# norabelrose/sparse-vae

Measured on AMD Instinct MI355X. Metric: training tokens/sec + ELBO match vs CPU ref, 512-tok seq, 1/2/4/8 MI355X, higher is better.
Workload: dtype bf16; 1 GPU; c2: TransformerVAE 6L d512 heads 8 seq 512, batch 64/GPU, dense attention, dropout 0.1, fwd+bwd+allreduce+clip+RAdam; model=TransformerVAE-6L-d512, global_batch=64, seq_len=512, parallelism=dp1

## Files before the change

sparse-vae_amd/csrc/gemm.hip:

```cpp
#include "common.h"
#include "../../include/svae.h"
#include <string.h>
#include <algorithm>
#include <vector>

using namespace svae;

namespace {

constexpr int BM = 128, BN = 128, BK = 64;
constexpr int TILE_BYTES = BM * BK * 2;

struct GP {
  const bf16* A; const bf16* B;
  long long lda, ldb, sA, sB;
  int M, N, K, splits, kchunk, tiles_n, tiles_m;
  void* C; long long ldc, sC;
  const float* bias;
  const float* resid; long long ldr;
  void* aux; long long ldaux;
  float alpha, drop_p;
  unsigned long long seed;
  const float* rot_tab; int rot_cols, rot_d, rot_seq;
  const int* labels; float* label_logit;
// ... 615 lines not shown

template <bool NT = false>
__device__ __forceinline__ void store_pair_bf16(bf16* row_base, int colbase, int ncols_left, const f32x4& x,
                                                const f32x4& y, int g) {
  const unsigned x0 = pack_bf16x2(x[0], x[1]), x1 = pack_bf16x2(x[2], x[3]);
  const unsigned y0 = pack_bf16x2(y[0], y[1]), y1 = pack_bf16x2(y[2], y[3]);
  const auto s0 = __builtin_amdgcn_permlane16_swap(x0, y0, false, false);
  const auto s1 = __builtin_amdgcn_permlane16_swap(x1, y1, false, false);
  const int c = colbase + ((g & 1) ? 16 : 0) + ((g & 2) ? 8 : 0);
  const u32x4 w = {s0[0], s1[0], s0[1], s1[1]};
  if (c + 8 <= ncols_left) {
    if constexpr (NT) __builtin_nontemporal_store(w, (u32x4*)(row_base + c));
    else *(u32x4*)(row_base + c) = w;
  } else if (c < ncols_left) *(u32x2*)(row_base + c) = (u32x2){w[0], w[1]};
}

template <bool B>
struct BoolC {
  static constexpr bool value = B;
};

template <int EPI>
__device__ __forceinline__ void g3_reg_epilogue(const GP& p, const f32x4 (&acc)[8][4], const float* sbias,
                                                const int* slabel, float* sstat, int m0, int n0, int bn, int batch,
                                                int split, int wr, int wc, int tid, int lane) {
  const long long cofs = (long long)batch * p.sC + split * p.slab;
  const int g = lane >> 4, li = lane & 15;
  f32x4 b4[4];
#pragma unroll
  for (int j = 0; j < 4; ++j) b4[j] = *(const f32x4*)(sbias + wc * 64 + j * 16 + 4 * g);
  f32x4 bl4[4];
#pragma unroll
  for (int j = 0; j < 4; ++j) bl4[j] = b4[j] * G3_LOG2E;
  int rofs[4] = {0, 0, 0, 0};
  bool rot_on[4] = {false, false, false, false};
  int pos = 0, pstep = 0;
  f32x4 cs_cur[4], cs_nxt[4];
  auto rot_load = [&](int ps, f32x4 (&cs)[4]) {
    const float* t = p.rot_tab + (long long)ps * p.rot_d;
#pragma unroll
    for (int j = 0; j < 4; ++j) cs[j] = rot_on[j] ? *(const f32x4*)(t + rofs[j]) : (f32x4){1.f, 0.f, 1.f, 0.f};
  };
  if constexpr (EPI == SVAE_EPI_ROTARY_BF16) {
#pragma unroll
    for (int j = 0; j < 4; ++j) {
      const int n = n0 + wc * 64 + j * 16 + 4 * g;
      rot_on[j] = n < p.rot_cols;
      rofs[j] = ((n % p.rot_d) >> 1) * 2;
    }
    pos = (m0 + wr * 128 + li) % p.rot_seq;
    pstep = 16 % p.rot_seq;
    rot_load(pos, cs_cur);
  }
#pragma unroll
  for (int i = 0; i < 8; ++i) {
    const int rl = wr * 128 + i * 16 + li, m = m0 + rl;
    f32x4 v[4];
#pragma unroll
    for (int j = 0; j < 4; ++j) v[j] = p.alpha * acc[i][j] + b4[j];
    if constexpr (EPI == SVAE_EPI_ROTARY_BF16) {
      int pn = pos + pstep;
      if (pn >= p.rot_seq) pn -= p.rot_seq;
      if (i + 1 < 8) rot_load(pn, cs_nxt);
#pragma unroll
      for (int j = 0; j < 4; ++j) {
        const f32x4 cs2 = cs_cur[j];
        const float a0 = v[j][0], b0 = v[j][1], a1 = v[j][2], b1 = v[j][3];
        v[j][0] = a0 * cs2[0] + (-b0) * cs2[1];
        v[j][1] = b0 * cs2[0] + a0 * cs2[1];
        v[j][2] = a1 * cs2[2] + (-b1) * cs2[3];
        v[j][3] = b1 * cs2[2] + a1 * cs2[3];
      }
      pos = pn;
      if (i + 1 < 8) {
#pragma unroll
        for (int j = 0; j < 4; ++j) cs_cur[j] = cs_nxt[j];
      }
    }
    {
      if constexpr (EPI == SVAE_EPI_GELU) {
        f32x4 gg[4], dg[4];
#pragma unroll
        for (int j = 0; j < 4; ++j)
#pragma unroll
          for (int e = 0; e < 4; e += 2) {
            f32x2 ge, de;
            gelu_pair2((f32x2){v[j][e], v[j][e + 1]}, ge, de);
            gg[j][e] = ge[0];
            gg[j][e + 1] = ge[1];
            dg[j][e] = de[0];
            dg[j][e + 1] = de[1];
          }
        store_rows_bf16<false>((bf16*)p.C + cofs, p.ldc, m0 + wr * 128 + i * 16, p.M, n0 + wc * 64, p.N, gg, g, li);
        store_rows_bf16<true>((bf16*)p.aux, p.ldaux, m0 + wr * 128 + i * 16, p.M, n0 + wc * 64, p.N, dg, g, li);
      } else if constexpr (EPI == SVAE_EPI_CE_PROB) {
        const float off = sstat[1024 + rl] * G3_LOG2E;
        const f32x2 sa2 = {p.alpha * G3_LOG2E, p.alpha * G3_LOG2E}, noff = {-off, -off};
        f32x2 se2 = {0.f, 0.f};
        auto body = [&](auto rag) {
          f32x4 xs[4];
#pragma unroll
          for (int j = 0; j < 4; ++j)
#pragma unroll
              for (int e = 0; e < 4; e += 2) {
                const f32x2 a2 = {acc[i][j][e], acc[i][j][e + 1]};
                const f32x2 c2 = (f32x2){bl4[j][e], bl4[j][e + 1]} + noff;
                const f32x2 t2 = a2 * sa2 + c2;
                f32x2 x = {__builtin_amdgcn_exp2f(t2[0]), __builtin_amdgcn_exp2f(t2[1])};
                if constexpr (decltype(rag)::value) {
                  const int n = n0 + wc * 64 + j * 16 + 4 * g + e;
                  if (n >= p.N) x[0] = 0.f;
                  if (n + 1 >= p.N) x[1] = 0.f;
                }
                xs[j][e] = x[0];
                xs[j][e + 1] = x[1];
                se2 += x;
              }
          store_rows_bf16<true>((bf16*)p.C + cofs, p.ldc, m0 + wr * 128 + i * 16, p.M, n0 + wc * 64, p.N, xs, g, li);
        };
        if (__builtin_amdgcn_readfirstlane((int)(n0 + wc * 64 + 64 > p.N))) body(BoolC<true>{});
        else body(BoolC<false>{});
        float se = sum_x16_x32(se2[0] + se2[1]);
        if (g == 0) sstat[rl * 4 + wc] = se;
      } else if (EPI != SVAE_EPI_CE_STATS || p.C) {
        store_rows_bf16<EPI == SVAE_EPI_CE_STATS>((bf16*)p.C + cofs, p.ldc, m0 + wr * 128 + i * 16, p.M, n0 + wc * 64,
                                                  p.N, v, g, li);
      }
    }
    if constexpr (EPI == SVAE_EPI_CE_STATS) {
      const bool ragged = n0 + wc * 64 + 64 > p.N;
      float mx = -INFINITY;
#pragma unroll
      for (int j = 0; j < 4; ++j)
#pragma unroll
        for (int e = 0; e < 4; ++e) {
          if (ragged && n0 + wc * 64 + j * 16 + 4 * g + e >= p.N) v[j][e] = -INFINITY;
          mx = fmaxf(mx, v[j][e]);
        }
      mx = max_x16_x32(mx);
      const float mc = mx == -INFINITY ? 0.f : mx * G3_LOG2E;
      float se = 0.f;
#pragma unroll
      for (int j = 0; j < 4; ++j)
#pragma unroll
        for (int e = 0; e < 4; ++e) se += __builtin_amdgcn_exp2f(fmaf(v[j][e], G3_LOG2E, -mc));
      se = sum_x16_x32(se);
      if (g == 0) {
        sstat[(rl * 4 + wc) * 2] = mx;
        sstat[(rl * 4 + wc) * 2 + 1] = se;
// ... 188 lines not shown
        const int n = nb + j * 16 + 4 * g;
        r[j] = (ld && m < p.M && n < p.N) ? *(const f32x4*)(src + (long long)m * lds_ + n) : (f32x4){0.f, 0.f, 0.f, 0.f};
      }
    };
    f32x4 cur[4], nxt[4];
    if constexpr (EPI != G3_EPI_SLAB) ld_row(0, cur);
#pragma unroll
    for (int i = 0; i < 8; ++i) {
      if (EPI != G3_EPI_SLAB && i + 1 < 8) ld_row(i + 1, nxt);
      const int m = m0 + wr * 128 + i * 16 + li;
      f32x4 x[4];
#pragma unroll
      for (int j = 0; j < 4; ++j) {
        const int n = nb + j * 16 + 4 * g;
        x[j] = p.alpha * acc[i][j] + b4[j];
        if constexpr (EPI == SVAE_EPI_DROPOUT_RESID) {
          if (p.drop_p > 0.f) dropout4(p, x[j], m, n);
        }
        if constexpr (EPI != G3_EPI_SLAB) x[j] += cur[j];
      }
      if constexpr (EPI == SVAE_EPI_F32_ACC) {
#pragma unroll
        for (int j = 0; j < 4; ++j) {
          const int n = nb + j * 16 + 4 * g;
          if (m < p.M && n < p.N) *(f32x4*)((float*)p.C + cofs + (long long)m * p.ldc + n) = x[j];
        }
      } else {
        store_rows_f32((float*)p.C + cofs, p.ldc, m0 + wr * 128 + i * 16, p.M, nb, p.N, x, g, li);
        if constexpr (EPI == SVAE_EPI_DROPOUT_RESID) {
          if (p.aux) store_rows_bf16<false>((bf16*)p.aux, p.ldaux, m0 + wr * 128 + i * 16, p.M, nb, p.N, x, g, li);
        } else if constexpr (EPI == SVAE_EPI_F32) {
          if (p.aux) {
            if (p.drop_p > 0.f) {
#pragma unroll
              for (int j = 0; j < 4; ++j) dropout4(p, x[j], m, nb + j * 16 + 4 * g);
            }
            store_rows_bf16<false>((bf16*)p.aux, p.ldaux, m0 + wr * 128 + i * 16, p.M, nb, p.N, x, g, li);
          }
        }
      }
      if (EPI != G3_EPI_SLAB && i + 1 < 8) {
#pragma unroll
        for (int j = 0; j < 4; ++j) cur[j] = nxt[j];
      }
    }
  }
}

struct G3Tile {
  int m0, n0, bn, batch, split, kbeg, kend, nk;
  const bf16* A; const bf16* B;
};

__device__ __forceinline__ G3Tile g3_tile(const GP& p, int t3) {
  G3Tile T;
  const int tiles = p.tn2 * p.tm2;
  const int z = t3 / tiles, t = t3 - z * tiles;
  T.batch = z / p.splits;
  T.split = z - T.batch * p.splits;
  int bm, bn;
  group_tile(t, p.tm2, p.tn2, p.group, bm, bn);
  T.bn = bn;
  T.m0 = bm * 256;
  T.n0 = bn * 256;
  T.kbeg = T.split * p.kchunk;
  T.kend = min(p.K, T.kbeg + p.kchunk);
  T.nk = T.kend > T.kbeg ? (T.kend - T.kbeg + 63) / 64 : 0;
  T.A = p.A + T.batch * p.sA;
  T.B = p.B + T.batch * p.sB;
  return T;
}

constexpr int G3_EPI_STORES = 16;

#ifdef SVAE_STAMPS
__device__ unsigned long long svae_stamps[8][96][3];
__device__ unsigned long long svae_rt[1024][2];
#define G3_STAMP(k) \
  do { if (blockIdx.x < 8 && tid == 0 && ntile < 96) svae_stamps[blockIdx.x][ntile][k] = __builtin_amdgcn_s_memtime(); } while (0)
#else
#define G3_STAMP(k) ((void)0)
#endif
#ifndef SVAE_KW_PRE
#define SVAE_KW_PRE 1
#endif

template <int EPI>
constexpr int g3_epi_vmem_ops() {
  switch (EPI) {
    case SVAE_EPI_BF16:
    case G3_EPI_BF16_DELTA:
    case SVAE_EPI_ROTARY_BF16:
    case SVAE_EPI_CE_STATS:
    case SVAE_EPI_ROWSCALE_GATHER:
    case SVAE_EPI_GELU_BWD:
      return 8 * 2;
    case SVAE_EPI_CE_PROB:
      return 8 * 2 + 1;
    case SVAE_EPI_GELU:
      return 8 * 2 * 2;
    case SVAE_EPI_F32:
    case SVAE_EPI_F32_ACC:
    case SVAE_EPI_DROPOUT_RESID:
    case G3_EPI_ACC_KW:
    case G3_EPI_F32_KW:
    case G3_EPI_SLAB:
      return 8 * 4;
    default:
      return 0;
  }
}

template <bool AT, bool BT, int EPI>
__device__ __forceinline__ void gemm256_run(const GP& p, int blk, int nwg, bool remap = true) {
  static_assert(g3_epi_vmem_ops<EPI>() >= G3_EPI_STORES, "the relaxed first wait would not cover the prefetch DMA");
  constexpr bool IS_KW = EPI == G3_EPI_ACC_KW || EPI == G3_EPI_F32_KW;
  __shared__ __attribute__((aligned(16))) char ring[2 * G3_STAGE + 2048 + 8192];
  float* sbias = (float*)(ring + 2 * G3_STAGE);
  int* slabel = (int*)(ring + 2 * G3_STAGE + 1024);
  float* sstat = (float*)(ring + 2 * G3_STAGE + 2048);
  const int tid = threadIdx.x, lane = tid & 63;
  const int wave = __builtin_amdgcn_readfirstlane(tid >> 6);
  const int wr = wave >> 2, wc = wave & 3;
  int bid = blk;
  if (remap && nwg >= 16) {
    const int q = nwg / 8, r = nwg % 8, xcd = bid % 8, idx = bid / 8;
    bid = (xcd < r ? xcd * (q + 1) : r * (q + 1) + (xcd - r) * q) + idx;
  }
  int t3 = bid;
  if (t3 >= p.total3) return;
  G3Tile T = g3_tile(p, t3);
  const G3Src sa = g3_src<AT>(p.lda, wave, lane), sb = g3_src<BT>(p.ldb, wave, lane);
  int g = 0;
  if (T.nk > 0) g3_issue<AT, BT>(p, T.A, T.B, sa, sb, T.m0, T.n0, T.kbeg, T.kend, ring, wave);

  bool relaxed = false;
  int ntile = 0;
  (void)ntile;
  while (true) {
    G3_STAMP(0);
    const int t3n = t3 + nwg;
    const bool has_next = t3n < p.total3;
    float rsum[4] = {0.f, 0.f, 0.f, 0.f};
    f32x4 acc[8][4];
#pragma unroll
    for (int i = 0; i < 8; ++i)
#pragma unroll
      for (int j = 0; j < 4; ++j) acc[i][j] = (f32x4){0.f, 0.f, 0.f, 0.f};

    const bool next_dma = has_next && g3_tile(p, t3n).nk > 0;
    for (int kt = 0; kt < T.nk; ++kt, ++g) {
      if (kt == 0 && relaxed) asm volatile("s_waitcnt vmcnt(%0)" ::"n"(G3_EPI_STORES) : "memory");
      else asm volatile("s_waitcnt vmcnt(0)" ::: "memory");
      __builtin_amdgcn_s_barrier();
      const char* la = ring + (g & 1) * G3_STAGE;
      const char* lb = la + G3_T;
      char* nxt = ring + ((g + 1) & 1) * G3_STAGE;
      const bool do_rs = AT && p.a_rowsum && T.bn < 2;
      const int ks0 = p.tn2 >= 2 ? T.bn : 0, ks1 = p.tn2 >= 2 ? T.bn + 1 : 2;
      const bool kw_pre = IS_KW && SVAE_KW_PRE && do_rs;
      float kw1 = 0.f;
      if (kw_pre) {
        const int kk = T.kbeg + kt * 64 + lane_id_fresh();
        const int off = kk < T.kend ? kk * 4 : 0x7FFFFFF0;
        const u32x4 kwr = buffer_rsrc(p.k_weight, 0x7FFFFFF0u);
        asm volatile("s_nop 4\n\tbuffer_load_dword %0, %1, %2, 0 offen" : "=&v"(kw1) : "v"(off), "s"(kwr) : "memory");
      }
      const bool late = (!IS_KW || kw_pre) && p.dma_stagger && wr == 1 && kt + 1 < T.nk;
      if (kt + 1 < T.nk) {
        if (!late) g3_issue<AT, BT>(p, T.A, T.B, sa, sb, T.m0, T.n0, T.kbeg + (kt + 1) * 64, T.kend, nxt, wave);
      } else if (next_dma) {
        const G3Tile TN = g3_tile(p, t3n);
        g3_issue<AT, BT>(p, TN.A, TN.B, sa, sb, TN.m0, TN.n0, TN.kbeg, TN.kend, nxt, wave);
      } else if (kw_pre) {
        const u32x4 rs = buffer_rsrc(p.A, 0x7FFFFFF0u);
#pragma unroll
        for (int i = 0; i < 8; ++i) dma16_lds(rs, nxt + (wave * 8 + i) * 1024, 0x7FFFFFF0);
      }
      bf16x8 a0[4][2], a1[4][2], b0[2][2], b1[2][2];
      auto rowsum2 = [&](const bf16x8 (&x)[2], const bf16x8 (&y)[2]) {
#pragma unroll
        for (int ks = 0; ks < 2; ++ks) {
          if (ks < ks0 || ks >= ks1) continue;
          f32x4 k0 = {1.f, 1.f, 1.f, 1.f}, k1 = k0;
          if constexpr (IS_KW) {
            if (kw_pre) {
              const int src0 = (32 * ks + 8 * (lane_id_fresh() >> 4)) * 4;
#pragma unroll
              for (int e = 0; e < 4; ++e) {
                k0[e] = __builtin_bit_cast(float, __builtin_amdgcn_ds_bpermute(src0 + 4 * e, __builtin_bit_cast(int, kw1)));
                k1[e] = __builtin_bit_cast(float, __builtin_amdgcn_ds_bpermute(src0 + 16 + 4 * e, __builtin_bit_cast(int, kw1)));
              }
            } else {
              const int kk = T.kbeg + kt * 64 + 32 * ks + 8 * (lane_id_fresh() >> 4);
              const int off = kk < T.kend ? kk * 4 : 0x7FFFFFF0;
              const u32x4 kwr = buffer_rsrc(p.k_weight, 0x7FFFFFF0u);
              asm volatile("s_nop 4\n\tbuffer_load_dwordx4 %0, %2, %3, 0 offen\n\t"
                           "buffer_load_dwordx4 %1, %2, %3, 0 offen offset:16\n\ts_waitcnt vmcnt(0)"
                           : "=&v"(k0), "=&v"(k1) : "v"(off), "s"(kwr) : "memory");
            }
          }
#pragma unroll
          for (int e = 0; e < 8; ++e) {
            const float kwe = e < 4 ? k0[e] : k1[e - 4];
            rsum[0] = fmaf((float)x[ks][e], kwe, rsum[0]);
            rsum[1] = fmaf((float)y[ks][e], kwe, rsum[1]);
          }
        }
      };
#pragma unroll
      for (int i = 0; i < 4; ++i)
#pragma unroll
        for (int ks = 0; ks < 2; ++ks) a0[i][ks] = g3_afrag<AT>(la, wr * 128 + i * 16, ks, lane);
#pragma unroll
      for (int j = 0; j < 2; ++j)
#pragma unroll
        for (int ks = 0; ks < 2; ++ks) b0[j][ks] = g3_bfrag<BT>(lb, wc * 64 + j * 16, ks, lane);
#pragma unroll
      for (int j = 0; j < 2; ++j)
#pragma unroll
        for (int ks = 0; ks < 2; ++ks) b1[j][ks] = g3_bfrag<BT>(lb, wc * 64 + 32 + j * 16, ks, lane);
#pragma unroll
      for (int ks = 0; ks < 2; ++ks)
#pragma unroll
        for (int i = 0; i < 4; ++i)
#pragma unroll
          for (int j = 0; j < 2; ++j) acc[i][j] = mfma16(b0[j][ks], a0[i][ks], acc[i][j]);
      if (late) {
        __builtin_amdgcn_sched_barrier(0);
        g3_issue<AT, BT>(p, T.A, T.B, sa, sb, T.m0, T.n0, T.kbeg + (kt + 1) * 64, T.kend, nxt, wave);
        __builtin_amdgcn_sched_barrier(0);
      }
      if constexpr (!AT) {
#pragma unroll
        for (int i = 0; i < 4; ++i)
#pragma unroll
          for (int ks = 0; ks < 2; ++ks) a1[i][ks] = g3_afrag<AT>(la, wr * 128 + 64 + i * 16, ks, lane);
      }
#pragma unroll
      for (int ks = 0; ks < 2; ++ks)
#pragma unroll
        for (int i = 0; i < 4; ++i)
#pragma unroll
          for (int j = 0; j < 2; ++j) acc[i][2 + j] = mfma16(b1[j][ks], a0[i][ks], acc[i][2 + j]);
      if constexpr (AT) {
        if (kw_pre) asm volatile("s_waitcnt vmcnt(8)" : "+v"(kw1) :: "memory");
        if (do_rs) {
          if (wc == 0) rowsum2(a0[0], a0[1]);
          else if (wc == 1) rowsum2(a0[2], a0[3]);
        }
#pragma unroll
        for (int i = 0; i < 4; ++i)
#pragma unroll
          for (int ks = 0; ks < 2; ++ks) a1[i][ks] = g3_afrag<AT>(la, wr * 128 + 64 + i * 16, ks, lane);
      }
#pragma unroll
      for (int ks = 0; ks < 2; ++ks)
#pragma unroll
        for (int i = 0; i < 4; ++i)
#pragma unroll
          for (int j = 0; j < 2; ++j) acc[4 + i][2 + j] = mfma16(b1[j][ks], a1[i][ks], acc[4 + i][2 + j]);
#pragma unroll
      for (int ks = 0; ks < 2; ++ks)
#pragma unroll
        for (int i = 0; i < 4; ++i)
#pragma unroll
          for (int j = 0; j < 2; ++j) acc[4 + i][j] = mfma16(b0[j][ks], a1[i][ks], acc[4 + i][j]);
      if constexpr (AT) {
        if (do_rs) {
          if (wc == 2) rowsum2(a1[0], a1[1]);
          else if (wc == 3) rowsum2(a1[2], a1[3]);
        }
      }
    }
    G3_STAMP(1);
    if (tid < 256) {
      const int n = T.n0 + tid, m = T.m0 + tid;
      sbias[tid] = (p.bias && n < p.N) ? p.bias[n] : 0.f;
      if (EPI == SVAE_EPI_CE_STATS || EPI == SVAE_EPI_CE_PROB || EPI == SVAE_EPI_ROWSCALE_GATHER)
        slabel[tid] = m < p.M ? p.labels[m] : 0;
      if (EPI == SVAE_EPI_CE_PROB) sstat[1024 + tid] = (m < p.M && p.labels[m] != 0) ? p.row_a[m] : INFINITY;
      if (EPI == SVAE_EPI_ROWSCALE_GATHER) sstat[1024 + tid] = m < p.M ? p.row_a[m] : 0.f;
      if (EPI == SVAE_EPI_ROWSCALE_GATHER) sstat[1280 + tid] = m < p.M ? p.row_b[m] : 0.f;
    }
    asm volatile("s_waitcnt lgkmcnt(0)" ::: "memory");
    __builtin_amdgcn_s_barrier();
    if constexpr (AT) {
      if (p.a_rowsum && T.bn < 2) {
#pragma unroll
        for (int h = 0; h < 2; ++h) {
          const float t = sum_x16_x32(rsum[h]);
          const int m = T.m0 + wr * 128 + (2 * wc + h) * 16 + (lane & 15);
          if ((lane >> 4) == 0 && m < p.M) atomicAdd(p.a_rowsum + m, t);
        }
      }
    }
    if constexpr (EPI == SVAE_EPI_BF16 || EPI == SVAE_EPI_GELU || EPI == SVAE_EPI_CE_STATS ||
                  EPI == SVAE_EPI_ROTARY_BF16 || EPI == SVAE_EPI_CE_PROB)
      g3_reg_epilogue<EPI>(p, acc, sbias, slabel, sstat, T.m0, T.n0, T.bn, T.batch, T.split, wr, wc, tid, lane);
    else if constexpr (EPI == SVAE_EPI_ROWSCALE_GATHER)
      g3_rowscale_gather_epilogue(p, acc, slabel, sstat + 1024, sstat + 1280, T.m0, T.n0, wr, wc, lane);
    else if constexpr (EPI == SVAE_EPI_F32 || EPI == SVAE_EPI_F32_ACC || EPI == SVAE_EPI_DROPOUT_RESID ||
                       EPI == SVAE_EPI_GELU_BWD || EPI == G3_EPI_BF16_DELTA)
      g3_reg_epilogue_ld<EPI>(p, acc, sbias, T.m0, T.n0, T.batch, T.split, wr, wc, lane);
    else if constexpr (EPI == G3_EPI_ACC_KW)
      g3_reg_epilogue_ld<SVAE_EPI_F32_ACC>(p, acc, sbias, T.m0, T.n0, T.batch, T.split, wr, wc, lane);
    else if constexpr (EPI == G3_EPI_F32_KW || EPI == G3_EPI_SLAB)
      g3_reg_epilogue_ld<G3_EPI_SLAB>(p, acc, sbias, T.m0, T.n0, T.batch, T.split, wr, wc, lane);
    else
      static_assert(EPI == G3_EPI_SLAB, "no gemm256 epilogue for this EPI");
    relaxed = p.relaxed && T.m0 + 256 <= p.M && T.n0 + 256 <= p.N;
    G3_STAMP(2);
    ++ntile;
    if (!has_next) break;
    const bool prefetched = T.nk > 0;
    t3 = t3n;
    T = g3_tile(p, t3);
    if (!prefetched && T.nk > 0)
      g3_issue<AT, BT>(p, T.A, T.B, sa, sb, T.m0, T.n0, T.kbeg, T.kend, ring + (g & 1) * G3_STAGE, wave);
  }
}

template <bool AT, bool BT, int EPI>
__global__ __launch_bounds__(512, 1) void gemm256_kernel(GP p) {
#ifdef SVAE_STAMPS
  if (threadIdx.x == 0 && blockIdx.x < 1024) svae_rt[blockIdx.x][0] = __builtin_amdgcn_s_memrealtime();
#endif
  gemm256_run<AT, BT, EPI>(p, blockIdx.x, gridDim.x);
#ifdef SVAE_STAMPS
  if (threadIdx.x == 0 && blockIdx.x < 1024) svae_rt[blockIdx.x][1] = __builtin_amdgcn_s_memrealtime();
#endif
}

struct GP2 {
  GP p[2];
  int nb0;
};

template <bool AT, bool BT, int EPI>
__global__ __launch_bounds__(512, 1) void gemm256_pair_kernel(GP2 q) {
  const int b = blockIdx.x;
  const int sel = b < q.nb0 ? 0 : 1;
  gemm256_run<AT, BT, EPI>(q.p[sel], sel ? b - q.nb0 : b, sel ? (int)gridDim.x - q.nb0 : q.nb0);
}

struct alignas(16) GPSlot {
  GP p;
};
struct alignas(16) GMap {
  int gemm, blk, nblk, pad;
};

template <class T>
__device__ __forceinline__ T load_uniform(const T* src) {
  static_assert(sizeof(T) % 4 == 0, "whole dwords");
  typedef const unsigned __attribute__((address_space(4))) * cu32p;
  struct W {
    unsigned w[sizeof(T) / 4];
  } r;
  const cu32p c = (cu32p)(uintptr_t)src;
#pragma unroll
  for (unsigned i = 0; i < sizeof(T) / 4; ++i) r.w[i] = c[i];
  return __builtin_bit_cast(T, r);
}

template <int EPI>
__global__ __launch_bounds__(512, 1) void gemm256_group_kernel(const GPSlot* __restrict__ tab,
                                                               const GMap* __restrict__ map) {
  const GMap e = load_uniform(map + blockIdx.x);
  if (e.gemm < 0) return;
// ... 547 lines not shown
      for (int k = 0; k < m; ++k)
        nb[c][k] = std::min(units[c][k], 1 + (int)((cap - m) * (work[c][k] / wsum)));
    place_blocks(idx[c], nb[c], map[c]);
  }
  const long long o_gp = sizeof(GroupHeader), o_ma = o_gp + (long long)n * sizeof(GPSlot);
  const long long o_mb = o_ma + (long long)map[0].size() * sizeof(GMap);
  const long long o_red = o_mb + (long long)map[1].size() * sizeof(GMap);
  const long long bytes = o_red + (long long)red.size() * sizeof(SlabRedSlot);
  if (bytes > table_bytes) return SVAE_EINVAL;
  std::vector<char> img((size_t)bytes, 0);
  const GroupHeader h{(unsigned long long)bytes, (unsigned long long)(uintptr_t)table, n, (int)map[0].size(),
                      (int)map[1].size(), (int)red.size()};
  memcpy(img.data(), &h, sizeof(h));
  memcpy(img.data() + o_gp, gp.data(), (size_t)n * sizeof(GPSlot));
  if (!map[0].empty()) memcpy(img.data() + o_ma, map[0].data(), map[0].size() * sizeof(GMap));
  if (!map[1].empty()) memcpy(img.data() + o_mb, map[1].data(), map[1].size() * sizeof(GMap));
  if (!red.empty()) memcpy(img.data() + o_red, red.data(), red.size() * sizeof(SlabRedSlot));
  hipStream_t s = (hipStream_t)stream;
  if (memcmp(table_host, img.data(), (size_t)bytes) != 0) {
    memcpy(table_host, img.data(), (size_t)bytes);
    if (hipMemcpyAsync(table, table_host, (size_t)bytes, hipMemcpyHostToDevice, s) != hipSuccess ||
        hipStreamSynchronize(s) != hipSuccess) {
      memset(table_host, 0, sizeof(GroupHeader));
      return SVAE_ELAUNCH;
    }
  }
  const char* t = (const char*)table;
  const GPSlot* tab = (const GPSlot*)(t + o_gp);
  if (!map[0].empty()) {
    hipLaunchKernelGGL((gemm256_group_kernel<SVAE_EPI_F32_ACC>), dim3((unsigned)map[0].size()), dim3(512), 0, s, tab,
                       (const GMap*)(t + o_ma));
    SVAE_LAUNCH_CHECK();
  }
  if (!map[1].empty()) {
    hipLaunchKernelGGL((gemm256_group_kernel<G3_EPI_SLAB>), dim3((unsigned)map[1].size()), dim3(512), 0, s, tab,
                       (const GMap*)(t + o_mb));
    SVAE_LAUNCH_CHECK();
    const long long rb = std::max(1LL, std::min(2048LL, (red_elems + 255) / 256));
    hipLaunchKernelGGL(slab_reduce_list_kernel, dim3((unsigned)rb), dim3(256), 0, s, (const SlabRedSlot*)(t + o_red),
                       (int)red.size());
    SVAE_LAUNCH_CHECK();
  }
  return SVAE_OK;
}

#ifdef SVAE_STAMPS
extern "C" __attribute__((visibility("default"))) int svae_debug_stamps(unsigned long long* host) {
  return hipMemcpyFromSymbol(host, HIP_SYMBOL(svae_stamps), sizeof(svae_stamps)) == hipSuccess ? 0 : -1;
}
extern "C" __attribute__((visibility("default"))) int svae_debug_rt(unsigned long long* host) {
  return hipMemcpyFromSymbol(host, HIP_SYMBOL(svae_rt), sizeof(svae_rt)) == hipSuccess ? 0 : -1;
}
extern "C" __attribute__((visibility("default"))) int svae_debug_stamps_clear() {
  static unsigned long long zeros[8 * 96 * 3];
  return hipMemcpyToSymbol(HIP_SYMBOL(svae_stamps), zeros, sizeof(zeros)) == hipSuccess ? 0 : -1;
}
#endif
```

sparse-vae_amd/csrc/attention.hip:

```cpp
#include "common.h"
#include <algorithm>
#include <type_traits>
#include "../../include/svae.h"

using namespace svae;

namespace {

struct AP {
  const bf16* q; const bf16* k; const bf16* v; bf16* o;
  long long sq, sk, sv, so, bq, bk, bv, bo;
  const unsigned char* pad; long long ldpad;
  float* lse;
  int B, H, Lq, Lk, hd, causal;
  float scale;
  const bf16* dout; long long sdo, bdo;
  const float* delta;
  float* dq; long long bdq;
  bf16* dk; bf16* dv; long long sdk, sdv, bdk, bdv;
  const float* rot; int rot_d;
  float* o32; long long so32, bo32;
  float* dq_part; void* dq_bf; long long ldq_bf;
  bf16* olo; long long solo, bolo;
  int window;
// ... 1416 lines not shown
  const u32x4 ors_o = buffer_rsrc(p.o + b * p.bo + (long long)h * p.hd, 0x7FFFFFF0u);
  const u32x4 ors_l = buffer_rsrc(p.olo ? p.olo + b * p.bolo + (long long)h * p.hd : p.o, 0x7FFFFFF0u);
  auto dik_issue = [&](int qb) {
    const int ln = lane_id_fresh();
    int oo[2], ol[2];
#pragma unroll
    for (int i = 0; i < 2; ++i) {
      const int r = 16 * (w - 4) + 8 * i + (ln >> 3), dd = 8 * (ln & 7);
      const bool ok = qb + r < p.Lq && dd < p.hd;
      oo[i] = ok ? ((qb + r) * (int)p.so + dd) * 2 : 0x7FFFFFF0;
      ol[i] = ok ? ((qb + r) * (int)p.solo + dd) * 2 : 0x7FFFFFF0;
    }
    dma16x2_lds(ors_o, dslot, oo[0], oo[1]);
    dma16x2_lds(ors_l, dslot + 2048, ol[0], ol[1]);
  };
  float* sscl = nullptr;
  if constexpr (HDC == 64) {
    sscl = (float*)(dslot - (w - 4) * 4096 + 4 * 4096);
    if (tid == 0) *sscl = p.scale;
  }
  auto dik_reduce = [&](int buf, int qb) {
    const int ln = lane_id_fresh();
    const int rl = ln >> 2, r = 16 * (w - 4) + rl, c0 = 2 * (ln & 3);
    const char* dimg = QO + buf * 2 * R::BYTES + R::BYTES;
    float sacc = 0.f;
#pragma unroll
    for (int hh = 0; hh < 2; ++hh) {
      const bf16x8 dv8 = *(const bf16x8*)(dimg + R::off(r, c0 + hh));
      const bf16x8 o8 = *(const bf16x8*)(dslot + rl * 128 + (c0 + hh) * 16);
      const bf16x8 l8 = *(const bf16x8*)(dslot + 2048 + rl * 128 + (c0 + hh) * 16);
#pragma unroll
      for (int e = 0; e < 8; ++e) sacc += ((float)o8[e] + (float)l8[e]) * (float)dv8[e];
    }
    sacc += __shfl_xor(sacc, 1);
    sacc += __shfl_xor(sacc, 2);
    if ((ln & 3) == 0) {
      dsh[buf * 64 + r] = sacc;
      if (qb + r < p.Lq) ((float*)p.delta)[((long long)b * p.H + h) * p.Lq + qb + r] = sacc;
    }
  };
  if (qt0 < nqt) fetch(qt0 * 64, 0);
  if (dik && w >= 4 && qt0 < nqt) dik_issue(qt0 * 64);
  asm volatile("s_waitcnt vmcnt(0)" ::: "memory");
  __syncthreads();
  if (dik) {
    if (w >= 4 && qt0 < nqt) dik_reduce(0, qt0 * 64);
    asm volatile("s_waitcnt lgkmcnt(0)" ::: "memory");
    __syncthreads();
  }
#pragma unroll
  for (int j = 0; j < 2; ++j)
#pragma unroll
    for (int kk = 0; kk < NKK; ++kk) asm volatile("" : "+v"(vf[j][kk]));

#ifdef SVAE_STAMPS
  { BWD8_T(t1); BWD8_ACC(0, t_start, t1); }
#endif
  for (int qt = qt0; qt < nqt; ++qt) {
#ifdef SVAE_STAMPS
    BWD8_T(ta);
    st_acc[7] += 1;
#endif
    const int buf = (qt - qt0) & 1;
    const int qb = qt * 64;
    const char* Qs = QO + buf * 2 * R::BYTES;
    const char* dOs = Qs + R::BYTES;
    const float* nl = cst + (buf * NWB + w) * 128;
    const bool rmw_t = rmw && qt < nqt_prev;
    if (rmw_t) {
      const int lf = lane_id_fresh();
      const bool qok = qb + 16 * dq_q16 + (lf & 15) < p.Lq;
      const int qrow = (qb + 16 * dq_q16 + (lf & 15)) * (int)ldp + 4 * (lf >> 4);
      const u32x4 prs4 = buffer_rsrc(part, 0x7FFFFFF0u);
      int ro[DQ_NT];
#pragma unroll
      for (int u = 0; u < DQ_NT; ++u) {
        const int d = 16 * (dq_u0 + u);
        ro[u] = (qok && d + 4 * (lf >> 4) < p.hd) ? (qrow + d) * 4 : 0x7FFFFFF0;
      }
      static_assert(DQ_NT == 2 || DQ_NT == 3, "dQ fragments per wave");
      if constexpr (DQ_NT == 2) dma16x2_lds(prs4, rslots + w * DQ_NT * 1024, ro[0], ro[1]);
      else dma16x3_lds(prs4, rslots + w * DQ_NT * 1024, ro[0], ro[1], ro[2]);
    }
    const bool direct_t = !(RMW && HDC == 96) && pk == 0 && qb + 64 <= p.dq_direct && qb + 64 <= k0 + BWD8_KEYS;
    const bool rot_t = direct_t && p.dq_bf && p.rot;
    if (rot_t) {
      const int lf = lane_id_fresh();
      const int q = qb + 16 * dq_q16 + (lf & 15);
      const bool qok = q < p.Lq;
      const u32x4 crs = buffer_rsrc(p.rot, 0x7FFFFFF0u);
      int co[DQ_NT];
#pragma unroll
      for (int u = 0; u < DQ_NT; ++u) {
        const int d = 16 * (dq_u0 + u) + 4 * (lf >> 4);
        co[u] = (qok && d < p.hd) ? (q * (p.rot_d / 2) + (h * p.hd + d) / 2) * 8 : 0x7FFFFFF0;
      }
      if constexpr (DQ_NT == 2) dma16x2_lds(crs, cslots + w * DQ_NT * 1024, co[0], co[1]);
      else dma16x3_lds(crs, cslots + w * DQ_NT * 1024, co[0], co[1], co[2]);
    }
    if (qt + 1 < nqt) fetch(qb + 64, buf ^ 1);
    if (dik && w >= 4 && qt + 1 < nqt) dik_issue(qb + 64);
    const float* dlp = dik ? dsh + buf * 64 : nl + 64;
    const bool live = (!p.causal || kw <= qb + 63) && qb < band_end && kw < p.Lk;
#ifdef SVAE_STAMPS
    if (live) st_acc[6] += 1;
#endif
    if (live && SVAE_BWD8_DIAG != 1) {
      const char* Kw = Ks + (wk >> 1) * R::BYTES;
      const bool edge = !keys_all_ok || qb + 64 > p.Lq || (p.causal && kw + 31 > qb) || qb + 63 >= band_end;
      const int qlim = min(p.Lq, band_end) - qb;
      constexpr int TPP = 2;
#pragma unroll
      for (int pass = 0; pass < 4 / TPP; ++pass) {
        bf16x8 kf[2][NKK];
#pragma unroll
        for (int j = 0; j < 2; ++j)
#pragma unroll
          for (int kk = 0; kk < NKK; ++kk) kf[j][kk] = *(const bf16x8*)(Kw + R::off(32 * (wk & 1) + 16 * j + li, g + 4 * kk));
        f32x4 s[2][TPP], dp[2][TPP];
#pragma unroll
        for (int th = 0; th < TPP; ++th) {
          const int t = pass * TPP + th;
          const f32x4 sl = *(const f32x4*)(nl + 16 * t + 4 * g) * -inv_scale;
          const f32x4 dl = -*(const f32x4*)(dlp + 16 * t + 4 * g);
          s[0][th] = sl; s[1][th] = sl;
          dp[0][th] = dl; dp[1][th] = dl;
          if (edge) {
#pragma unroll
            for (int j = 0; j < 2; ++j) {
              const int kmin = p.causal ? kw + 16 * j + li - qb : -0x40000000;
              const unsigned kbad = key_ok[j] ? 0u : 1u;
#pragma unroll
              for (int r = 0; r < 4; ++r) {
                const int ql = 16 * t + 4 * g + r;
                s[j][th][r] = (kbad | (unsigned)(ql >= qlim) | (unsigned)(ql < kmin)) ? -INFINITY : s[j][th][r];
              }
            }
          }
#pragma unroll
          for (int k2 = 0; k2 < NKK; ++k2) {
            const bf16x8 qa = *(const bf16x8*)(Qs + R::off(16 * t + li, g + 4 * k2));
            const bf16x8 oa = *(const bf16x8*)(dOs + R::off(16 * t + li, g + 4 * k2));
            s[0][th] = mfma16(qa, kf[0][k2], s[0][th]);
            s[1][th] = mfma16(qa, kf[1][k2], s[1][th]);
            dp[0][th] = mfma16(oa, vf[0][k2], dp[0][th]);
            dp[1][th] = mfma16(oa, vf[1][k2], dp[1][th]);
          }
        }
#pragma unroll
        for (int j = 0; j < 2; ++j)
#pragma unroll
          for (int th = 0; th < TPP; ++th)
#pragma unroll
            for (int r = 0; r < 4; ++r) {
              const float pr = __builtin_amdgcn_exp2f(s[j][th][r] * c);
              s[j][th][r] = pr;
              dp[j][th][r] = pr * dp[j][th][r];
            }
#pragma unroll
        for (int k2 = 0; k2 < TPP / 2; ++k2) {
          const int kk = pass * (TPP / 2) + k2;
          const bf16x8 pf0 = pack8(s[0][2 * k2], s[0][2 * k2 + 1]), pf1 = pack8(s[1][2 * k2], s[1][2 * k2 + 1]);
          const bf16x8 df0 = pack8(dp[0][2 * k2], dp[0][2 * k2 + 1]), df1 = pack8(dp[1][2 * k2], dp[1][2 * k2 + 1]);
          const int rq = 4 * g + (li >> 2);
#pragma unroll
          for (int u = 0; u < NT; ++u) {
            const int uu = 4 * u + (li & 3);
            const int pitch = 16 * u < 64 ? 128 : 64;
            const int lo = R::uoff(rq, uu);
            const int ro = 32 * kk * pitch;
            const lds_char* po = lds_ptr(dOs) + lo + ro;
            const lds_char* pq = lds_ptr(Qs) + lo + ro;
            const bf16x8 ao = cat44(lds_read_tr3(po), lds_read_tr3(po + 16 * pitch));
            dv[0][u] = mfma16(ao, pf0, dv[0][u]);
            dv[1][u] = mfma16(ao, pf1, dv[1][u]);
            const bf16x8 aq = cat44(lds_read_tr3(pq), lds_read_tr3(pq + 16 * pitch));
            dk[0][u] = mfma16(aq, df0, dk[0][u]);
            dk[1][u] = mfma16(aq, df1, dk[1][u]);
          }
        }
#pragma unroll
        for (int j = 0; j < 2; ++j)
#pragma unroll
          for (int th = 0; th < TPP; ++th)
            *(bf16x4*)(dSs + TS::uoff(32 * wk + 16 * j + li, 4 * (pass * TPP + th) + g)) =
                (bf16x4){f2bf(dp[j][th][0]), f2bf(dp[j][th][1]), f2bf(dp[j][th][2]), f2bf(dp[j][th][3])};
      }
    } else {
      const bf16x4 z = {f2bf(0.f), f2bf(0.f), f2bf(0.f), f2bf(0.f)};
#pragma unroll
      for (int j = 0; j < 2; ++j)
#pragma unroll
        for (int t = 0; t < 4; ++t) *(bf16x4*)(dSs + TS::uoff(32 * wk + 16 * j + li, 4 * t + g)) = z;
    }
    asm volatile("s_waitcnt lgkmcnt(0)" ::: "memory");
#ifdef SVAE_STAMPS
    BWD8_T(tb);
    BWD8_ACC(1, ta, tb);
#endif
    __builtin_amdgcn_s_barrier();
    asm volatile("" ::: "memory");
    if (dik && w >= 4 && qt + 1 < nqt) {
      asm volatile("s_waitcnt vmcnt(0)" ::: "memory");
      dik_reduce(buf ^ 1, qb + 64);
    }
#ifdef SVAE_STAMPS
    BWD8_T(tc);
    BWD8_ACC(2, tb, tc);
#endif
    f32x4 dq[DQ_NT];
#pragma unroll
    for (int u = 0; u < DQ_NT; ++u) dq[u] = (f32x4){0.f, 0.f, 0.f, 0.f};
    const int kvis = p.causal ? min(BWD8_KEYS, qb + 64 - k0) : min(BWD8_KEYS, p.Lk - k0);
    {
      const int q4 = 8 * g + (li >> 2);
      const int uq = 4 * dq_q16 + (li & 3);
      const lds_char* sp0 = lds_ptr(dSs) + TS::uoff(q4, uq);
      const lds_char* sp4 = lds_ptr(dSs) + TS::uoff(q4 + 4, uq);
      const lds_char* kp0[DQ_NT];
      const lds_char* kp4[DQ_NT];
#pragma unroll
      for (int u = 0; u < DQ_NT; ++u) {
        const int uk = 4 * (dq_u0 + u) + (li & 3);
        kp0[u] = lds_ptr(Ks) + R::uoff(q4, uk);
        kp4[u] = lds_ptr(Ks) + R::uoff(q4 + 4, uk);
      }
#pragma unroll
      for (int kk = 0; kk < BWD8_KEYS / 32; ++kk) {
        if (32 * kk >= kvis || SVAE_BWD8_DIAG == 1) break;
        const int so = kk * 32 * TS::PITCH;
        const bf16x8 a = cat44(lds_read_tr3(sp0 + so), lds_read_tr3(sp4 + so));
#pragma unroll
        for (int u = 0; u < DQ_NT; ++u) {
          const int pitch = 16 * (dq_u0 + u) < 64 ? 128 : 64;
          const int ko = (kk >> 1) * R::BYTES + (kk & 1) * 32 * pitch;
          const bf16x8 bk = cat44(lds_read_tr3(kp0[u] + ko), lds_read_tr3(kp4[u] + ko));
          dq[u] = mfma16(bk, a, dq[u]);
        }
      }
    }
    if (rmw_t || rot_t) {
      if (qt + 1 < nqt) {
        if (dik && w >= 4) asm volatile("s_waitcnt vmcnt(%0)" ::"n"(QO_PW + 6) : "memory");
        else asm volatile("s_waitcnt vmcnt(%0)" ::"n"(QO_PW + 2) : "memory");
      } else {
        asm volatile("s_waitcnt vmcnt(0)" ::: "memory");
      }
    }
    if (rmw_t) {
      const lds_char* sl = lds_ptr(rslots + w * DQ_NT * 1024) + 16 * lane_id_fresh();
#pragma unroll
      for (int u = 0; u < DQ_NT; ++u) dq[u] += *(const f32x4*)(sl + 1024 * u);
    }
    if (direct_t) {
      const int lf = lane_id_fresh();
      const int q = qb + 16 * dq_q16 + (lf & 15);
      const bool qok = q < p.Lq;
#pragma unroll
      for (int u = 0; u < DQ_NT; ++u) {
        const int d = 16 * (dq_u0 + u) + 4 * (lf >> 4);
        const bool ok = qok && d < p.hd;
        float scl = p.scale;
        if constexpr (HDC == 64) scl = *(volatile const float*)sscl;
        f32x4 v = dq[u] * scl;
        if (p.dq_bf) {
          if (p.rot) {
            const f32x4 cs = *(const f32x4*)(lds_ptr(cslots + w * DQ_NT * 1024) + 16 * lf + 1024 * u);
            const float a0 = v[0], b0 = v[1], a1 = v[2], b1 = v[3];
            v[0] = a0 * cs[0] + b0 * cs[1];
            v[1] = -a0 * cs[1] + b0 * cs[0];
            v[2] = a1 * cs[2] + b1 * cs[3];
            v[3] = -a1 * cs[3] + b1 * cs[2];
          }
          const bf16x4 pd = {f2bf(v[0]), f2bf(v[1]), f2bf(v[2]), f2bf(v[3])};
          __builtin_amdgcn_raw_buffer_store_b64(__builtin_bit_cast(u32x2, pd), drs,
                                                ok ? (q * (int)p.ldq_bf + d) * 2 : 0x7FFFFFF0, 0, 0);
        } else {
          __builtin_amdgcn_raw_buffer_store_b128(__builtin_bit_cast(u32x4, v), drs, ok ? (q * (int)ldp + d) * 4 : 0x7FFFFFF0,
                                                 0, 0);
        }
      }
    } else {
      const bool qok = qb + 16 * dq_q16 + li < p.Lq;
      const int qrow = (qb + 16 * dq_q16 + li) * (int)ldp + 4 * g;
#pragma unroll
      for (int u = 0; u < DQ_NT; ++u) {
        const int d = 16 * (dq_u0 + u);
        const int off = (qok && d + 4 * g < p.hd) ? (qrow + d) * 4 : 0x7FFFFFF0;
        __builtin_amdgcn_raw_buffer_store_b128(__builtin_bit_cast(u32x4, dq[u]), prs, off, 0, 0);
      }
    }
// ... 584 lines not shown
```

Measured before the change: 2.829 million tokens/s.

## Prefetch epilogue side data via async LDS DMA during mainloop in seam GEMMs

For non-transposed-A GEMMs with CE_PROB, GELU, GELU_BWD and rotary epilogues, the bias, label and row-stat loads that fed the epilogue are now issued as buffer-to-LDS DMA at the first k-step. This replaces the scalar global loads and extra barrier that ran between the mainloop and the epilogue. Next-tile coordinates are computed once at the last k-step and reused when the loop advances. The CE_PROB label masking moves into the epilogue as a precomputed per-row offset. The changes are meant to hide the loop-to-epilogue seam latency, but they rely on the mainloop's later vmcnt waits and barriers to order the side DMA, and only apply when nk >= 2.

```diff
diff --git a/sparse-vae_amd/csrc/gemm.hip b/sparse-vae_amd/csrc/gemm.hip
--- a/sparse-vae_amd/csrc/gemm.hip
+++ b/sparse-vae_amd/csrc/gemm.hip
@@ -691,6 +691,14 @@
     pstep = 16 % p.rot_seq;
     rot_load(pos, cs_cur);
   }
+  float ceoff[8];
+  if constexpr (EPI == SVAE_EPI_CE_PROB) {
+#pragma unroll
+    for (int i = 0; i < 8; ++i) {
+      const int rl = wr * 128 + i * 16 + li;
+      ceoff[i] = (slabel[rl] != 0 ? sstat[1024 + rl] : INFINITY) * G3_LOG2E;
+    }
+  }
 #pragma unroll
   for (int i = 0; i < 8; ++i) {
     const int rl = wr * 128 + i * 16 + li, m = m0 + rl;
@@ -733,7 +741,7 @@
         store_rows_bf16<false>((bf16*)p.C + cofs, p.ldc, m0 + wr * 128 + i * 16, p.M, n0 + wc * 64, p.N, gg, g, li);
         store_rows_bf16<true>((bf16*)p.aux, p.ldaux, m0 + wr * 128 + i * 16, p.M, n0 + wc * 64, p.N, dg, g, li);
       } else if constexpr (EPI == SVAE_EPI_CE_PROB) {
-        const float off = sstat[1024 + rl] * G3_LOG2E;
+        const float off = ceoff[i];
         const f32x2 sa2 = {p.alpha * G3_LOG2E, p.alpha * G3_LOG2E}, noff = {-off, -off};
         f32x2 se2 = {0.f, 0.f};
         auto body = [&](auto rag) {
@@ -1028,17 +1036,27 @@
   const bf16* A; const bf16* B;
 };
 
-__device__ __forceinline__ G3Tile g3_tile(const GP& p, int t3) {
-  G3Tile T;
+struct G3Coord {
+  int bm, bn, batch, split;
+};
+
+__device__ __forceinline__ G3Coord g3_coord(const GP& p, int t3) {
+  G3Coord c;
   const int tiles = p.tn2 * p.tm2;
   const int z = t3 / tiles, t = t3 - z * tiles;
-  T.batch = z / p.splits;
-  T.split = z - T.batch * p.splits;
-  int bm, bn;
-  group_tile(t, p.tm2, p.tn2, p.group, bm, bn);
-  T.bn = bn;
-  T.m0 = bm * 256;
-  T.n0 = bn * 256;
+  c.batch = z / p.splits;
+  c.split = z - c.batch * p.splits;
+  group_tile(t, p.tm2, p.tn2, p.group, c.bm, c.bn);
+  return c;
+}
+
+__device__ __forceinline__ G3Tile g3_tile(const GP& p, const G3Coord& c) {
+  G3Tile T;
+  T.batch = c.batch;
+  T.split = c.split;
+  T.bn = c.bn;
+  T.m0 = c.bm * 256;
+  T.n0 = c.bn * 256;
   T.kbeg = T.split * p.kchunk;
   T.kend = min(p.K, T.kbeg + p.kchunk);
   T.nk = T.kend > T.kbeg ? (T.kend - T.kbeg + 63) / 64 : 0;
@@ -1047,10 +1065,13 @@
   return T;
 }
 
+__device__ __forceinline__ G3Tile g3_tile(const GP& p, int t3) { return g3_tile(p, g3_coord(p, t3)); }
+
 constexpr int G3_EPI_STORES = 16;
 
 #ifdef SVAE_STAMPS
-__device__ unsigned long long svae_stamps[8][96][3];
+constexpr int G3_NSTAMP = 5;
+__device__ unsigned long long svae_stamps[8][96][G3_NSTAMP];
 __device__ unsigned long long svae_rt[1024][2];
 #define G3_STAMP(k) \
   do { if (blockIdx.x < 8 && tid == 0 && ntile < 96) svae_stamps[blockIdx.x][ntile][k] = __builtin_amdgcn_s_memtime(); } while (0)
@@ -1087,10 +1108,25 @@
   }
 }
 
+template <int EPI>
+__device__ __forceinline__ void g3_side_issue(const GP& p, int m0, int n0, float* sbias, int* slabel, float* sstat,
+                                              int wave) {
+  const int l = wave * 64 + lane_id_fresh();
+  const int on = (p.bias && n0 + l < p.N) ? (n0 + l) * 4 : 0x7FFFFFF0;
+  dma4_lds(buffer_rsrc(p.bias, 0x7FFFFFF0u), sbias + wave * 64, on);
+  if constexpr (EPI == SVAE_EPI_CE_PROB) {
+    const int om = m0 + l < p.M ? (m0 + l) * 4 : 0x7FFFFFF0;
+    dma4_lds(buffer_rsrc(p.labels, 0x7FFFFFF0u), slabel + wave * 64, om);
+    dma4_lds(buffer_rsrc(p.row_a, 0x7FFFFFF0u), sstat + 1024 + wave * 64, om);
+  }
+}
+
 template <bool AT, bool BT, int EPI>
 __device__ __forceinline__ void gemm256_run(const GP& p, int blk, int nwg, bool remap = true) {
   static_assert(g3_epi_vmem_ops<EPI>() >= G3_EPI_STORES, "the relaxed first wait would not cover the prefetch DMA");
   constexpr bool IS_KW = EPI == G3_EPI_ACC_KW || EPI == G3_EPI_F32_KW;
+  constexpr bool SEAM = !AT && (EPI == SVAE_EPI_CE_PROB || EPI == SVAE_EPI_GELU || EPI == SVAE_EPI_GELU_BWD ||
+                                EPI == SVAE_EPI_ROTARY_BF16);
   __shared__ __attribute__((aligned(16))) char ring[2 * G3_STAGE + 2048 + 8192];
   float* sbias = (float*)(ring + 2 * G3_STAGE);
   int* slabel = (int*)(ring + 2 * G3_STAGE + 1024);
@@ -1110,6 +1146,7 @@
   int g = 0;
   if (T.nk > 0) g3_issue<AT, BT>(p, T.A, T.B, sa, sb, T.m0, T.n0, T.kbeg, T.kend, ring, wave);
 
+  G3Coord cn = {0, 0, 0, 0};
   bool relaxed = false;
   int ntile = 0;
   (void)ntile;
@@ -1124,11 +1161,15 @@
 #pragma unroll
       for (int j = 0; j < 4; ++j) acc[i][j] = (f32x4){0.f, 0.f, 0.f, 0.f};
 
-    const bool next_dma = has_next && g3_tile(p, t3n).nk > 0;
+    bool next_dma = false;
+    if constexpr (!SEAM) next_dma = has_next && g3_tile(p, t3n).nk > 0;
+    const bool side_dma = SEAM && T.nk >= 2;
     for (int kt = 0; kt < T.nk; ++kt, ++g) {
       if (kt == 0 && relaxed) asm volatile("s_waitcnt vmcnt(%0)" ::"n"(G3_EPI_STORES) : "memory");
       else asm volatile("s_waitcnt vmcnt(0)" ::: "memory");
       __builtin_amdgcn_s_barrier();
+      if (kt == 0) G3_STAMP(4);
+      if (side_dma && kt == 0 && wave < 4) g3_side_issue<EPI>(p, T.m0, T.n0, sbias, slabel, sstat, wave);
       const char* la = ring + (g & 1) * G3_STAGE;
       const char* lb = la + G3_T;
       char* nxt = ring + ((g + 1) & 1) * G3_STAGE;
@@ -1145,9 +1186,15 @@
       const bool late = (!IS_KW || kw_pre) && p.dma_stagger && wr == 1 && kt + 1 < T.nk;
       if (kt + 1 < T.nk) {
         if (!late) g3_issue<AT, BT>(p, T.A, T.B, sa, sb, T.m0, T.n0, T.kbeg + (kt + 1) * 64, T.kend, nxt, wave);
+      } else if (SEAM) {
+        if (has_next) {
+          cn = g3_coord(p, t3n);
+          const G3Tile TN = g3_tile(p, cn);
+          if (TN.nk > 0) g3_issue<AT, BT>(p, TN.A, TN.B, sa, sb, TN.m0, TN.n0, TN.kbeg, TN.kend, nxt, wave);
+        }
       } else if (next_dma) {
-        const G3Tile TN = g3_tile(p, t3n);
-        g3_issue<AT, BT>(p, TN.A, TN.B, sa, sb, TN.m0, TN.n0, TN.kbeg, TN.kend, nxt, wave);
+        const G3Tile TD = g3_tile(p, t3n);
+        g3_issue<AT, BT>(p, TD.A, TD.B, sa, sb, TD.m0, TD.n0, TD.kbeg, TD.kend, nxt, wave);
       } else if (kw_pre) {
         const u32x4 rs = buffer_rsrc(p.A, 0x7FFFFFF0u);
 #pragma unroll
@@ -1250,17 +1297,19 @@
       }
     }
     G3_STAMP(1);
-    if (tid < 256) {
-      const int n = T.n0 + tid, m = T.m0 + tid;
-      sbias[tid] = (p.bias && n < p.N) ? p.bias[n] : 0.f;
-      if (EPI == SVAE_EPI_CE_STATS || EPI == SVAE_EPI_CE_PROB || EPI == SVAE_EPI_ROWSCALE_GATHER)
-        slabel[tid] = m < p.M ? p.labels[m] : 0;
-      if (EPI == SVAE_EPI_CE_PROB) sstat[1024 + tid] = (m < p.M && p.labels[m] != 0) ? p.row_a[m] : INFINITY;
-      if (EPI == SVAE_EPI_ROWSCALE_GATHER) sstat[1024 + tid] = m < p.M ? p.row_a[m] : 0.f;
-      if (EPI == SVAE_EPI_ROWSCALE_GATHER) sstat[1280 + tid] = m < p.M ? p.row_b[m] : 0.f;
-    }
-    asm volatile("s_waitcnt lgkmcnt(0)" ::: "memory");
-    __builtin_amdgcn_s_barrier();
+    if (!side_dma) {
+      if (tid < 256) {
+        const int n = T.n0 + tid, m = T.m0 + tid;
+        sbias[tid] = (p.bias && n < p.N) ? p.bias[n] : 0.f;
+        if (EPI == SVAE_EPI_CE_STATS || EPI == SVAE_EPI_CE_PROB || EPI == SVAE_EPI_ROWSCALE_GATHER)
+          slabel[tid] = m < p.M ? p.labels[m] : 0;
+        if (EPI == SVAE_EPI_CE_PROB || EPI == SVAE_EPI_ROWSCALE_GATHER) sstat[1024 + tid] = m < p.M ? p.row_a[m] : 0.f;
+        if (EPI == SVAE_EPI_ROWSCALE_GATHER) sstat[1280 + tid] = m < p.M ? p.row_b[m] : 0.f;
+      }
+      asm volatile("s_waitcnt lgkmcnt(0)" ::: "memory");
+      __builtin_amdgcn_s_barrier();
+    }
+    G3_STAMP(3);
     if constexpr (AT) {
       if (p.a_rowsum && T.bn < 2) {
 #pragma unroll
@@ -1291,7 +1340,8 @@
     if (!has_next) break;
     const bool prefetched = T.nk > 0;
     t3 = t3n;
-    T = g3_tile(p, t3);
+    if (SEAM && prefetched) T = g3_tile(p, cn);
+    else T = g3_tile(p, t3);
     if (!prefetched && T.nk > 0)
       g3_issue<AT, BT>(p, T.A, T.B, sa, sb, T.m0, T.n0, T.kbeg, T.kend, ring + (g & 1) * G3_STAGE, wave);
   }
@@ -1945,7 +1995,7 @@
   return hipMemcpyFromSymbol(host, HIP_SYMBOL(svae_rt), sizeof(svae_rt)) == hipSuccess ? 0 : -1;
 }
 extern "C" __attribute__((visibility("default"))) int svae_debug_stamps_clear() {
-  static unsigned long long zeros[8 * 96 * 3];
+  static unsigned long long zeros[8 * 96 * G3_NSTAMP];
   return hipMemcpyToSymbol(HIP_SYMBOL(svae_stamps), zeros, sizeof(zeros)) == hipSuccess ? 0 : -1;
 }
 #endif
```

New measurement: 2.835 million tokens/s, median of 3. No clear change (+0.2%).

## Keep K fragments register-resident and software-pipeline LDS reads in attention backward

Applied to the files above, without the earlier changes.

For head dim 64, the attention backward kernel now loads the K fragments into registers once before the q-tile loop instead of reloading them from LDS on every pass. The S/dP, dV/dK and dQ inner loops are restructured to issue LDS reads one step ahead (double-buffered Q/dO/K fragments), with sched_barrier fences so they overlap with MFMA work. The aim is to cut LDS traffic and hide LDS latency behind matrix instructions. The cost is higher VGPR pressure, which may lower occupancy or cause spills, plus a more complex code path.

```diff
diff --git a/sparse-vae_amd/csrc/attention.hip b/sparse-vae_amd/csrc/attention.hip
--- a/sparse-vae_amd/csrc/attention.hip
+++ b/sparse-vae_amd/csrc/attention.hip
@@ -1492,6 +1492,19 @@
   for (int j = 0; j < 2; ++j)
 #pragma unroll
     for (int kk = 0; kk < NKK; ++kk) asm volatile("" : "+v"(vf[j][kk]));
+  constexpr bool KF_RES = HDC == 64;
+  bf16x8 kfr[2][NKK];
+  if constexpr (KF_RES) {
+    const char* Kw = Ks + (wk >> 1) * R::BYTES;
+#pragma unroll
+    for (int j = 0; j < 2; ++j)
+#pragma unroll
+      for (int kk = 0; kk < NKK; ++kk) kfr[j][kk] = *(const bf16x8*)(Kw + R::off(32 * (wk & 1) + 16 * j + li, g + 4 * kk));
+#pragma unroll
+    for (int j = 0; j < 2; ++j)
+#pragma unroll
+      for (int kk = 0; kk < NKK; ++kk) asm volatile("" : "+v"(kfr[j][kk]));
+  }
 
 #ifdef SVAE_STAMPS
   { BWD8_T(t1); BWD8_ACC(0, t_start, t1); }
@@ -1546,10 +1559,104 @@
     if (live) st_acc[6] += 1;
 #endif
     if (live && SVAE_BWD8_DIAG != 1) {
-      const char* Kw = Ks + (wk >> 1) * R::BYTES;
+      [[maybe_unused]] const char* Kw = Ks + (wk >> 1) * R::BYTES;
       const bool edge = !keys_all_ok || qb + 64 > p.Lq || (p.causal && kw + 31 > qb) || qb + 63 >= band_end;
       const int qlim = min(p.Lq, band_end) - qb;
       constexpr int TPP = 2;
+      if constexpr (KF_RES) {
+        bf16x8 qa[TPP][NKK], oa[TPP][NKK], ao[NT], aq[NT];
+        f32x4 sl[TPP], dl[TPP];
+        auto rd_s = [&](int t, int th) {
+          sl[th] = *(const f32x4*)(nl + 16 * t + 4 * g);
+          dl[th] = *(const f32x4*)(dlp + 16 * t + 4 * g);
+#pragma unroll
+          for (int k2 = 0; k2 < NKK; ++k2) {
+            qa[th][k2] = *(const bf16x8*)(Qs + R::off(16 * t + li, g + 4 * k2));
+            oa[th][k2] = *(const bf16x8*)(dOs + R::off(16 * t + li, g + 4 * k2));
+          }
+        };
+        auto rd_t = [&](int kk, int u) {
+          const int lo = R::uoff(4 * g + (li >> 2), 4 * u + (li & 3)) + 32 * kk * 128;
+          const lds_char* po = lds_ptr(dOs) + lo;
+          const lds_char* pq = lds_ptr(Qs) + lo;
+          ao[u] = cat44(lds_read_tr3(po), lds_read_tr3(po + 16 * 128));
+          aq[u] = cat44(lds_read_tr3(pq), lds_read_tr3(pq + 16 * 128));
+        };
+        rd_s(0, 0);
+        rd_s(1, 1);
+        __builtin_amdgcn_sched_barrier(0);
+#pragma unroll
+        for (int pass = 0; pass < 4 / TPP; ++pass) {
+          f32x4 s[2][TPP], dp[2][TPP];
+          if (pass > 0) {
+            rd_s(pass * TPP + 1, 1);
+            __builtin_amdgcn_sched_barrier(0);
+          }
+#pragma unroll
+          for (int th = 0; th < TPP; ++th) {
+            const int t = pass * TPP + th;
+            const f32x4 sn = sl[th] * -inv_scale;
+            const f32x4 dn = -dl[th];
+            s[0][th] = sn; s[1][th] = sn;
+            dp[0][th] = dn; dp[1][th] = dn;
+            if (edge) {
+#pragma unroll
+              for (int j = 0; j < 2; ++j) {
+                const int kmin = p.causal ? kw + 16 * j + li - qb : -0x40000000;
+                const unsigned kbad = key_ok[j] ? 0u : 1u;
+#pragma unroll
+                for (int r = 0; r < 4; ++r) {
+                  const int ql = 16 * t + 4 * g + r;
+                  s[j][th][r] = (kbad | (unsigned)(ql >= qlim) | (unsigned)(ql < kmin)) ? -INFINITY : s[j][th][r];
+                }
+              }
+            }
+#pragma unroll
+            for (int k2 = 0; k2 < NKK; ++k2) {
+              s[0][th] = mfma16(qa[th][k2], kfr[0][k2], s[0][th]);
+              s[1][th] = mfma16(qa[th][k2], kfr[1][k2], s[1][th]);
+              dp[0][th] = mfma16(oa[th][k2], vf[0][k2], dp[0][th]);
+              dp[1][th] = mfma16(oa[th][k2], vf[1][k2], dp[1][th]);
+            }
+            __builtin_amdgcn_sched_barrier(0);
+            if (th == 0) {
+              rd_t(pass, 0);
+              rd_t(pass, 1);
+              __builtin_amdgcn_sched_barrier(0);
+            }
+          }
+#pragma unroll
+          for (int j = 0; j < 2; ++j)
+#pragma unroll
+            for (int th = 0; th < TPP; ++th)
+#pragma unroll
+              for (int r = 0; r < 4; ++r) {
+                const float pr = __builtin_amdgcn_exp2f(s[j][th][r] * c);
+                s[j][th][r] = pr;
+                dp[j][th][r] = pr * dp[j][th][r];
+              }
+          const bf16x8 pf0 = pack8(s[0][0], s[0][1]), pf1 = pack8(s[1][0], s[1][1]);
+          const bf16x8 df0 = pack8(dp[0][0], dp[0][1]), df1 = pack8(dp[1][0], dp[1][1]);
+#pragma unroll
+          for (int j = 0; j < 2; ++j)
+#pragma unroll
+            for (int th = 0; th < TPP; ++th)
+              *(bf16x4*)(dSs + TS::uoff(32 * wk + 16 * j + li, 4 * (pass * TPP + th) + g)) =
+                  (bf16x4){f2bf(dp[j][th][0]), f2bf(dp[j][th][1]), f2bf(dp[j][th][2]), f2bf(dp[j][th][3])};
+          __builtin_amdgcn_sched_barrier(0);
+#pragma unroll
+          for (int u = 0; u < NT; ++u) {
+            dv[0][u] = mfma16(ao[u], pf0, dv[0][u]);
+            dv[1][u] = mfma16(ao[u], pf1, dv[1][u]);
+            dk[0][u] = mfma16(aq[u], df0, dk[0][u]);
+            dk[1][u] = mfma16(aq[u], df1, dk[1][u]);
+            __builtin_amdgcn_sched_barrier(0);
+            if (u + 2 < NT) rd_t(pass, u + 2);
+            else if (u + 2 == NT && pass + 1 < 4 / TPP) rd_s((pass + 1) * TPP, 0);
+            __builtin_amdgcn_sched_barrier(0);
+          }
+        }
+      } else {
 #pragma unroll
       for (int pass = 0; pass < 4 / TPP; ++pass) {
         bf16x8 kf[2][NKK];
@@ -1626,6 +1733,7 @@
             *(bf16x4*)(dSs + TS::uoff(32 * wk + 16 * j + li, 4 * (pass * TPP + th) + g)) =
                 (bf16x4){f2bf(dp[j][th][0]), f2bf(dp[j][th][1]), f2bf(dp[j][th][2]), f2bf(dp[j][th][3])};
       }
+      }
     } else {
       const bf16x4 z = {f2bf(0.f), f2bf(0.f), f2bf(0.f), f2bf(0.f)};
 #pragma unroll
@@ -1665,6 +1773,30 @@
         kp0[u] = lds_ptr(Ks) + R::uoff(q4, uk);
         kp4[u] = lds_ptr(Ks) + R::uoff(q4 + 4, uk);
       }
+      if constexpr (KF_RES) {
+        bf16x8 af[2], bkf[2][DQ_NT];
+        auto rd_q = [&](int kk, int st) {
+          const int so = kk * 32 * TS::PITCH, ko = (kk >> 1) * R::BYTES + (kk & 1) * 32 * 128;
+          af[st] = cat44(lds_read_tr3(sp0 + so), lds_read_tr3(sp4 + so));
+#pragma unroll
+          for (int u = 0; u < DQ_NT; ++u) bkf[st][u] = cat44(lds_read_tr3(kp0[u] + ko), lds_read_tr3(kp4[u] + ko));
+        };
+        const int nkk = SVAE_BWD8_DIAG == 1 ? 0 : (kvis + 31) >> 5;
+        if (nkk > 0) {
+          rd_q(0, 0);
+          rd_q(1, 1);
+          __builtin_amdgcn_sched_barrier(0);
+#pragma unroll
+          for (int kk = 0; kk < BWD8_KEYS / 32; ++kk) {
+            if ((kk & 1) == 0 && kk >= nkk) break;
+#pragma unroll
+            for (int u = 0; u < DQ_NT; ++u) dq[u] = mfma16(bkf[kk & 1][u], af[kk & 1], dq[u]);
+            __builtin_amdgcn_sched_barrier(0);
+            if (kk + 2 < BWD8_KEYS / 32) rd_q(kk + 2, kk & 1);
+            __builtin_amdgcn_sched_barrier(0);
+          }
+        }
+      } else {
 #pragma unroll
       for (int kk = 0; kk < BWD8_KEYS / 32; ++kk) {
         if (32 * kk >= kvis || SVAE_BWD8_DIAG == 1) break;
@@ -1677,6 +1809,7 @@
           const bf16x8 bk = cat44(lds_read_tr3(kp0[u] + ko), lds_read_tr3(kp4[u] + ko));
           dq[u] = mfma16(bk, a, dq[u]);
         }
+      }
       }
     }
     if (rmw_t || rot_t) {
```

New measurement: 2.792 million tokens/s before, 2.786 million tokens/s after. About the same (-0.2%).
